# simzero/cudaParticlesFoam

Measured on AMD Instinct MI355X. Metric: Mparticle-steps/s, higher is better.
Workload: dtype f64

## Files before the change

### cudaparticlesfoam_amd/csrc/cpf_stream.hip

```cpp
#include "cpf_stream_ops.h"

#include <hip/hip_ext.h>

#include <type_traits>

namespace cpf {

#ifndef CPF_STREAM_SLOTS
#define CPF_STREAM_SLOTS 6
#endif
#ifndef CPF_STREAM_SLOTS_FIXED
#define CPF_STREAM_SLOTS_FIXED 9
#endif
#ifndef CPF_STREAM_WAVES
#define CPF_STREAM_WAVES 7
#endif
constexpr int kStreamSlots = CPF_STREAM_SLOTS;
constexpr int kStreamSlotsFixed = CPF_STREAM_SLOTS_FIXED;
constexpr int kSlotStride = 8;
static_assert(kStreamSlots >= 4 && kStreamSlots <= 32 && kStreamSlotsFixed >= 4 && kStreamSlotsFixed <= 32, "slots");
#ifndef CPF_STREAM_GATHER_LANES
#define CPF_STREAM_GATHER_LANES 32
#endif
constexpr int kStreamGatherLanes = CPF_STREAM_GATHER_LANES;
#ifndef CPF_STREAM_PAIRED
#define CPF_STREAM_PAIRED 0
#endif
#ifndef CPF_STREAM_INROUND
#define CPF_STREAM_INROUND 0
#endif
#ifndef CPF_STREAM_HIT_POOL
#define CPF_STREAM_HIT_POOL 40
#endif
constexpr int kVertexTets = 12;
#ifndef CPF_VERTEX_BLOCKS
#define CPF_VERTEX_BLOCKS 4
#endif
#ifndef CPF_VERTEX_PICK_UNROLL
#define CPF_VERTEX_PICK_UNROLL 12
#endif
constexpr int kVertexBlocks = CPF_VERTEX_BLOCKS;
constexpr int kStreamSparsePerCell = 8;
constexpr int kSitOut = INT32_MIN + 7;

struct StreamKernArgs {
    double *x, *y, *z; int32_t* cell; const int64_t* gid; double* vel; int64_t n; double dt, sigma; uint32_t step0; int nCyc;
    uint32_t seed; MeshView m; unsigned long long* counters; StreamArgs sa;
};
static_assert(offsetof(StreamKernArgs, x) == 0 && offsetof(StreamKernArgs, cell) == 24, "kernarg_cloud_ptrs reads bytes 0..31");
constexpr int kKernArgHitSpill = (int)(offsetof(StreamKernArgs, sa) + offsetof(StreamArgs, hitSpill));
constexpr int kKernArgZBad = (int)(offsetof(StreamKernArgs, sa) + offsetof(StreamArgs, zBad));
constexpr int kKernArgGid = (int)offsetof(StreamKernArgs, gid), kKernArgSigma = (int)offsetof(StreamKernArgs, sigma);
constexpr int kKernArgStep0 = (int)offsetof(StreamKernArgs, step0), kKernArgSeed = (int)offsetof(StreamKernArgs, seed);
#ifndef CPF_STREAM_BROWN_KERNARG
#define CPF_STREAM_BROWN_KERNARG 1
#endif

#ifndef CPF_STREAM_L1_ZERO_SKIP
#define CPF_STREAM_L1_ZERO_SKIP 1
#endif
#ifndef CPF_STREAM_LAZY_USED
#define CPF_STREAM_LAZY_USED 1
#endif
#ifndef CPF_STREAM_BOX_SPARSE
#define CPF_STREAM_BOX_SPARSE 1
#endif
#ifndef CPF_STREAM_FLAT_KICK
#define CPF_STREAM_FLAT_KICK 0
#endif
#ifndef CPF_STREAM_FLAT_ZERO_SKIP
#define CPF_STREAM_FLAT_ZERO_SKIP 0
#endif
#ifndef CPF_STREAM_FLAT_Z
#define CPF_STREAM_FLAT_Z 1
#endif
#ifndef CPF_STREAM_SLOTS_BOX
#define CPF_STREAM_SLOTS_BOX 9
#endif
#ifndef CPF_STREAM_SLOTS_BOX_B
#define CPF_STREAM_SLOTS_BOX_B 12
#endif
#ifndef CPF_STREAM_WAVES_BOX_B
#define CPF_STREAM_WAVES_BOX_B 6
#endif
#ifndef CPF_STREAM_WAVES_BOX
#define CPF_STREAM_WAVES_BOX 6
#endif
#ifndef CPF_STREAM_WAVES_B1
#define CPF_STREAM_WAVES_B1 5
#endif
#ifndef CPF_STREAM_WAVES_L2
#define CPF_STREAM_WAVES_L2 6
#endif
#ifndef CPF_STREAM_WAVES_B0
#define CPF_STREAM_WAVES_B0 7
#endif
#ifndef CPF_STREAM_HIT_POOL_B0
#define CPF_STREAM_HIT_POOL_B0 18
#endif
#ifndef CPF_STREAM_WAVES_FLAT
#define CPF_STREAM_WAVES_FLAT CPF_STREAM_WAVES
#endif
#ifndef CPF_STREAM_WAVES_FLAT_BODY
#define CPF_STREAM_WAVES_FLAT_BODY 0
#endif
template <bool BROWNIAN, bool STORE_VEL, bool STATS, int LOOKUP>
struct StreamOccupancy {
    static constexpr bool kMixed = LOOKUP == 2 || LOOKUP == 3 || LOOKUP == 5 || LOOKUP == 11;
    static constexpr int waves = (STORE_VEL || STATS) ? 1 : (LOOKUP == 4 ? (BROWNIAN ? 4 : 5) : (BROWNIAN ? (kMixed ? 5 : ((LOOKUP == 6 || LOOKUP == 11) ? CPF_STREAM_WAVES_BOX_B : (LOOKUP == 1 ? CPF_STREAM_WAVES_B1 : CPF_STREAM_WAVES_B0))) : (LOOKUP == 2 ? CPF_STREAM_WAVES_L2 : ((kMixed && LOOKUP != 11) ? 6 : ((LOOKUP == 6 || LOOKUP == 11) ? CPF_STREAM_WAVES_BOX : (LOOKUP == 8 ? CPF_STREAM_WAVES_FLAT : CPF_STREAM_WAVES))))));
};

template <bool BROWNIAN, bool REFLECT, bool STORE_VEL, bool STATS, int LOOKUP, bool VERTEX, bool ZSET = false>
__device__ __forceinline__ void stream_body(
    const int64_t* __restrict__ gid, double* __restrict__ vel, int64_t n, double dt, double sigma, uint32_t step0,
    int nCyc, uint32_t seed, const MeshView& m, unsigned long long* __restrict__ counters, const StreamArgs& sa, const VertexField& vf) {
#ifndef CPF_STREAM_SLOTS_BROWN
#define CPF_STREAM_SLOTS_BROWN 10
#endif
    constexpr int NS = (LOOKUP == 0 || LOOKUP == 5 || LOOKUP == 8) ? kStreamSlots : ((LOOKUP == 6 || LOOKUP == 11) ? (BROWNIAN ? CPF_STREAM_SLOTS_BOX_B : CPF_STREAM_SLOTS_BOX) : (BROWNIAN && LOOKUP == 1 ? CPF_STREAM_SLOTS_BROWN : kStreamSlotsFixed));
    constexpr bool BOX = LOOKUP == 6 || LOOKUP == 11;
    constexpr int kStride = BOX ? 4 : kSlotStride;
    constexpr unsigned kRecBytes = 32u * kStride;
    constexpr unsigned ALL = NS == 32 ? 0xFFFFFFFFu : ((1u << NS) - 1u);
    __shared__ double4 slots[NS][kStride];
    __shared__ unsigned sCnt[4];
#ifndef CPF_STREAM_HIT_REGS_L2
#define CPF_STREAM_HIT_REGS_L2 0
#endif
    constexpr bool HIT_IN_REGS = !BROWNIAN && (LOOKUP != 2 || CPF_STREAM_HIT_REGS_L2);
    constexpr bool kInRound = CPF_STREAM_INROUND == 2 || (CPF_STREAM_INROUND == 1 && BROWNIAN);
    static_assert(!(kInRound && (LOOKUP == 2 || LOOKUP == 3 || LOOKUP == 5 || LOOKUP == 11)), "in-round reflection knows neither face groups nor two-record cells");
    constexpr int kPool = HIT_IN_REGS ? 1 : ((LOOKUP == 2 || LOOKUP == 3 || LOOKUP == 5 || LOOKUP == 11) ? 16 : ((BROWNIAN && LOOKUP == 0) ? CPF_STREAM_HIT_POOL_B0 : CPF_STREAM_HIT_POOL));
    static_assert(!ZSET || ((LOOKUP == 8 || LOOKUP == 9) && !BROWNIAN && !VERTEX), "settled z: the flat walk without the kick or the vertex advect");
    __shared__ double sLane[ZSET ? 2 : 3][64];
    __shared__ double sPool[3][kPool];
    __shared__ unsigned sPoolUsed;
    __shared__ double sPre[ZSET ? 160 : (BROWNIAN ? 288 : 224)];
    __shared__ double sCone[VERTEX ? kVertexBlocks : 1][VERTEX ? kVertexTets * 10 : 1];
    double(*sE)[64] = sLane;
    const int lane = threadIdx.x;
    const unsigned ul = threadIdx.x;
    const unsigned preBase = uniform32(lds_addr(sPre));
    const unsigned slotBase = uniform32(lds_addr(slots));
    const int tpc = sa.tilesPerChunk;
    constexpr bool LOOKUP_FIXED = LOOKUP != 0 && LOOKUP != 5 && LOOKUP != 8;
    constexpr bool FLAT = LOOKUP == 8 || LOOKUP == 9;
    const bool zKeep = ZSET || (FLAT && CPF_STREAM_FLAT_Z != 0 && sa.zSettled != 0);
    auto park = [&](const D3& e) __attribute__((always_inline)) {
        sE[0][lane] = e.x; sE[1][lane] = e.y;
        if (!ZSET) sE[2][lane] = e.z;
    };
    auto parked = [&]() __attribute__((always_inline)) -> D3 {
        if (ZSET) return {sE[0][lane], sE[1][lane], 0.0};
        return {sE[0][lane], sE[1][lane], sE[2][lane]};
    };
    constexpr bool mixed = LOOKUP == 2 || LOOKUP == 3 || LOOKUP == 5 || LOOKUP == 11;
    constexpr bool bigCells = LOOKUP == 2;
    constexpr int kGatherAhead = LOOKUP == 4 ? 3 : 0;
    const bool zFold = !BOX && BROWNIAN && REFLECT && m.zThin != 0;
    const bool zLast = !FLAT && !BROWNIAN && m.zPairLast != 0;
    const bool flatKick = zFold && m.zSide0 != 0;
    const unsigned nTiles = (unsigned)((n + 63) >> 6);
    const unsigned nFull = (unsigned)(n >> 6), nTail = (unsigned)n & 63u;
    const unsigned big = sa.bigChunks;
    const unsigned nChunks = big + (nTiles - big * (unsigned)tpc);
    auto chunk_first = [&](unsigned c) -> unsigned {
        return c < big ? c * (unsigned)tpc : big * (unsigned)tpc + (c - big);
    };
    auto chunk_tiles = [&](unsigned c, unsigned firstTile) -> int {
        if (c >= nChunks) return 0;
        const unsigned k = nTiles - firstTile;
        const unsigned want = c < big ? (unsigned)tpc : 1u;
        return (int)(k < want ? k : want);
    };
    auto chunk_of = [&](unsigned j) -> unsigned {
        const unsigned long long c = (unsigned long long)(blockIdx.x & (kStreamGroups - 1)) + (unsigned long long)kStreamGroups * j;
        return c < (unsigned long long)nChunks ? (unsigned)c : nChunks;
    };
    StepStats st = {0, 0, 0, 0};
#ifdef CPF_STREAM_TIMELINE
    const uint64_t tl0 = __builtin_amdgcn_s_memrealtime();
    unsigned tlTiles = 0, tlRounds = 0;
    unsigned tlWaitRec = 0, tlWaitEnd = 0, tlMissRounds = 0;
    unsigned long long* const tlH = (!STORE_VEL && vel != nullptr && (sa.debug & 4)) ? reinterpret_cast<unsigned long long*>(vel) + 8 * 16384 : nullptr;
    unsigned tlVis = 0, tlRoundIdx = 0;
#endif

    for (unsigned k = blockIdx.x; k < (unsigned)kStreamGroups; k += gridDim.x)
        if (lane == 0) sa.grabNext[k * kStreamCounterStride] = 0u;
    const unsigned grp = blockIdx.x & (kStreamGroups - 1);
    unsigned* const myGrab = sa.grab + grp * kStreamCounterStride;

    auto prefetch = [&](unsigned t, const CloudPtrs& cp) __attribute__((always_inline)) -> int {
        double* const x = cp.x; double* const y = cp.y; double* const z = cp.z; int32_t* const cell = cp.cell;
        t = uniform32(t);
        const int64_t b = (int64_t)t * 64;
        unsigned ul = threadIdx.x;
        asm volatile("" : "+v"(ul));
        if (t < nFull) {
            const char* s1 = (ul < 32u ? reinterpret_cast<const char*>(x + b) : reinterpret_cast<const char*>(y + b)) + (ul & 31u) * 16u;
            glds16(s1, preBase);
            if (zKeep) {
                if (ul < 16u) glds16(reinterpret_cast<const char*>(cell + b) + ul * 16u, preBase + 1024u);
            } else if (ul < 48u) {
                const char* s2 = ul < 32u ? reinterpret_cast<const char*>(z + b) + ul * 16u
                                          : reinterpret_cast<const char*>(cell + b) + (ul - 32u) * 16u;
                glds16(s2, preBase + 1024u);
            }
            if (BROWNIAN) {
                const int64_t* const g = CPF_STREAM_BROWN_KERNARG ? static_cast<const int64_t*>(kernarg_pointer<kKernArgGid>()) : gid;
                if (g != nullptr) {
                    if (ul < 32u) glds16(reinterpret_cast<const char*>(g + b) + ul * 16u, preBase + 1792u);
                    return 3;
                }
            }
            return 2;
        }
        const unsigned lim = nTail - 1u;
        const unsigned l = ul < lim ? ul : lim;
        if (zKeep) {
            const double vx = (x + b)[l], vy = (y + b)[l];
            const int vc = (cell + b)[l];
            sPre[ul] = vx; sPre[64 + ul] = vy;
            reinterpret_cast<int*>(sPre + 128)[ul] = vc;
        } else {
        const double vx = (x + b)[l], vy = (y + b)[l], vz = (z + b)[l];
        const int vc = (cell + b)[l];
        sPre[ul] = vx; sPre[64 + ul] = vy; sPre[128 + ul] = vz;
        reinterpret_cast<int*>(sPre + 192)[ul] = vc;
        }
        if (BROWNIAN) {
            const int64_t* const g = CPF_STREAM_BROWN_KERNARG ? static_cast<const int64_t*>(kernarg_pointer<kKernArgGid>()) : gid;
            if (g != nullptr) reinterpret_cast<int64_t*>(sPre + 224)[ul] = (g + b)[l];
        }
        return 0;
    };

    unsigned got0 = 0;
    if (lane == 0) got0 = grab_sync(myGrab);
    const unsigned chunk0 = chunk_of(uniform32(got0));
    if (chunk_tiles(chunk0, chunk_first(chunk0)) > 0) {
        int tagv = -1;
        unsigned fifo = 0;

        unsigned tile = chunk_first(chunk0);
        int tilesLeft = chunk_tiles(chunk0, tile);
        (void)prefetch(tile, kernarg_cloud_ptrs());
        wait_vmcnt<0>();

        bool havePrev = false;
        unsigned rtile = 0;
        double rvx = 0, rvy = 0, rvz = 0;
        bool ralive = false;
        int rc = 0;
        unsigned rlim = 63;

        for (;;) {
            tile = uniform32(tile);
            const unsigned plim = tile < nFull ? 63u : nTail - 1u;
            double px = sPre[ul], py = sPre[64 + ul], pz = 0.0;
            int pc;
            if (zKeep) pc = reinterpret_cast<const int*>(sPre + 128)[ul];
            else { pz = sPre[128 + ul]; pc = reinterpret_cast<const int*>(sPre + 192)[ul]; }
            uint64_t pid = 0;
            if (BROWNIAN) {
                const bool haveIds = (CPF_STREAM_BROWN_KERNARG ? kernarg_pointer<kKernArgGid>() : (void*)gid) != nullptr;
                pid = haveIds ? (uint64_t) reinterpret_cast<const int64_t*>(sPre + 224)[ul] : (uint64_t)tile * 64 + ul;
            }
            if (ul > plim || pc < 0) pc = CPF_CELL_FROZEN;
            if (FLAT && !ZSET && !zKeep && ballot64(pc >= 0 && !(fabs(pz) <= 1.7976931348623157e308)) != 0ull) {
                unsigned* const bad = static_cast<unsigned*>(kernarg_pointer<kKernArgZBad>());
                if (bad != nullptr && lane == 0) *bad = 1u;
            }

            int cur = pc;
            int key2 = 0, carNext = 0, carBest = -1;
            double carDT = 2.0;
            D3 S_ = {px, py, pz}, v = {0, 0, 0};
            const uint64_t id = pid;

            unsigned ntile = 0;
            int ntilesLeft = 0;

            auto hook = [&](const D3& prev) __attribute__((always_inline)) -> int {
                int younger = 0;
                __builtin_amdgcn_sched_barrier(0);
                if (tilesLeft > 1) {
                    ntile = tile + 1;
                    ntilesLeft = tilesLeft - 1;
                } else {
                    unsigned got = 0;
                    if (lane == 0) got = grab_sync(myGrab);
                    const unsigned nxt = chunk_of(uniform32(got));
                    ntile = chunk_first(nxt);
                    ntilesLeft = chunk_tiles(nxt, ntile);
                }
                const CloudPtrs cp = kernarg_cloud_ptrs();
                double* const x = cp.x; double* const y = cp.y; double* const z = cp.z; int32_t* const cell = cp.cell;
                if (havePrev && !(sa.debug & 1)) {
                    const int64_t b = (int64_t)uniform32(rtile) * 64;
                    if (STORE_VEL && ralive) {
                        double* vv = vel + 3 * b;
                        async_store(vv, ul * 24u, rvx); async_store(vv + 1, ul * 24u, rvy); async_store(vv + 2, ul * 24u, rvz);
                    }
                    if (ul <= rlim) {
                        async_store(x + b, ul * 8u, prev.x); async_store(y + b, ul * 8u, prev.y);
                        if (!zKeep) async_store(z + b, ul * 8u, prev.z);
                        async_store(cell + b, ul * 4u, rc);
                    }
                    younger += zKeep ? 3 : 4;
                }
                if (ntilesLeft > 0 && !(sa.debug & 2)) younger += prefetch(ntile, cp);
                __builtin_amdgcn_sched_barrier(0);
                return younger;
            };

            bool busy = false;
            bool zUnclear = false;
            int token = INT32_MIN, h = 0, j = 0;
            int hitAt = -1;
            D3 hitReg = {0, 0, 0};
            auto park_hit = [&](const D3& Hp) __attribute__((always_inline)) {
                if (HIT_IN_REGS) { hitReg = Hp; return; }
                if (hitAt < 0) hitAt = (int)atomicAdd(&sPoolUsed, 1u);
                if (hitAt < kPool) { sPool[0][hitAt] = Hp.x; sPool[1][hitAt] = Hp.y; sPool[2][hitAt] = Hp.z; }
                else {
                    double* sp = static_cast<double*>(kernarg_pointer<kKernArgHitSpill>()) + (size_t)blockIdx.x * kStreamHitSpillDoubles;
                    async_store(sp, ul * 8u, Hp.x); async_store(sp + 64, ul * 8u, Hp.y); async_store(sp + 128, ul * 8u, Hp.z);
                }
            };

            auto cycle_begin = [&](int c) __attribute__((always_inline)) {
                if (cur < 0) cur = CPF_CELL_FROZEN;
                busy = cur >= 0;
                token = INT32_MIN; h = 0; j = 0;
                if (bigCells) key2 = 0;
                if (!HIT_IN_REGS && REFLECT) { hitAt = -1; if (lane == 0) sPoolUsed = 0u; }
                zUnclear = false;
                if (STATS && busy) ++st.steps;
                if (VERTEX) {
                    bool slow = busy;
#if defined(CPF_VERTEX_AB) && CPF_VERTEX_AB == 1
                    if (busy) { const double4 u = m.U[cur]; v = {u.x, u.y, u.z}; slow = false; }
#endif
                    if (vf.tetsPerCell == kVertexTets) {
                        unsigned long long todo = ballot64(slow);
                        while (todo != 0ull) {
                            int myBlock = -1;
                            __syncthreads();
#pragma unroll
                            for (int q = 0; q < kVertexBlocks; ++q) {
                                if (todo != 0ull) {
                                    const int ck = __builtin_amdgcn_readlane(cur, __ffsll((long long)todo) - 1);
                                    const bool mine = slow && cur == ck;
                                    if (mine) myBlock = q;
                                    if (lane < 5 * kVertexTets) {
                                        const int tk = lane / 5, piece = lane - 5 * tk;
                                        const double2 row = reinterpret_cast<const double2*>(vf.cone + kConeDoubles * ((int64_t)ck * kVertexTets + tk))[piece];
                                        reinterpret_cast<double2*>(&sCone[q][0] + 10 * tk)[piece] = row;
                                    }
                                    todo &= ~ballot64(mine);
                                }
                            }
                            __syncthreads();
                            if (myBlock >= 0) {
                                const double4 ap = vf.apex[cur];
                                const D3 A = {ap.x, ap.y, ap.z};
                                const D3 r = {S_.x - A.x, S_.y - A.y, S_.z - A.z};
                                int cand = 0;
                                double candMin = -1e300;
                                const double* blk = &sCone[myBlock][0];
#pragma unroll CPF_VERTEX_PICK_UNROLL
                                for (int k = 0; k < kVertexTets; ++k) {
                                    const double2* g = reinterpret_cast<const double2*>(blk + 10 * k);
                                    const double2 g01 = g[0], g23 = g[1], g45 = g[2], g67 = g[3], g89 = g[4];
                                    const double cb = fma(g23.x, r.z, fma(g01.y, r.y, g01.x * r.x)), cc = fma(g45.y, r.z, fma(g45.x, r.y, g23.y * r.x));
                                    const double cd = fma(g89.x, r.z, fma(g67.y, r.y, g67.x * r.x));
                                    const double mm = fmin(cb, fmin(cc, cd));
                                    if (mm > candMin) { candMin = mm; cand = k; }
                                }
#if defined(CPF_VERTEX_AB) && CPF_VERTEX_AB == 2
                                { const double4 u = m.U[cur]; v = {u.x + 1e-300 * cand, u.y, u.z}; slow = false; }
#else
                                D3 vv;
                                if (vertex_velocity_in_tet(vf, S_, A, (int64_t)cur * kVertexTets + cand, vv)) { v = vv; slow = false; }
#endif
                            }
                        }
                    }
                    if (slow) (void)vertex_velocity(vf, S_, cur, v);
                }
            };

            auto round = [&](bool hookDue, bool cycleStart, int c) __attribute__((always_inline)) {
#ifdef CPF_STREAM_TIMELINE
                ++tlRounds;
                bool tlSat = false;
#endif
                const unsigned long long busyMask = ballot64(busy);
                const D3 Epre = parked();
                const int lk = (bigCells && key2 != 0) ? key2 : cur;
                int myslot = -1;
                unsigned used = 0;
                unsigned long long missLanes = busyMask;
                if (LOOKUP_FIXED) {
                    const int cell0 = __builtin_amdgcn_readlane(lk, __ffsll((long long)busyMask) - 1);
                    const unsigned long long in0 = __builtin_amdgcn_uicmp((unsigned)lk, (unsigned)cell0, 32 ) & busyMask;
                    if (in0 == busyMask) {
                        const unsigned long long hitTag = __builtin_amdgcn_uicmp((unsigned)tagv, (unsigned)cell0, 32 ) & ALL;
                        if (hitTag != 0ull) {
                            myslot = __ffsll((long long)hitTag) - 1;
                            used = (unsigned)hitTag;
                            missLanes = 0ull;
                        }
                    } else {
#if CPF_STREAM_LAZY_USED
                        unsigned long long eqs[NS];
#pragma unroll
                        for (int k = 0; k < NS; ++k) {
                            const int tk = __builtin_amdgcn_readlane(tagv, k);
                            eqs[k] = __builtin_amdgcn_uicmp((unsigned)lk, (unsigned)tk, 32 );
                            asm("v_cndmask_b32_e64 %0, %1, %2, %3" : "=v"(myslot) : "v"(myslot), "n"(k), "s"(eqs[k]));
                        }
                        missLanes = ballot64(myslot < 0) & busyMask;
                        if (missLanes != 0ull) {
#pragma unroll
                            for (int k = 0; k < NS; ++k) used |= ((eqs[k] & busyMask) != 0ull ? 1u : 0u) << k;
                        }
#else
#pragma unroll
                        for (int k = 0; k < NS; ++k) {
                            const int tk = __builtin_amdgcn_readlane(tagv, k);
                            const unsigned long long eqK = __builtin_amdgcn_uicmp((unsigned)lk, (unsigned)tk, 32 );
                            const unsigned long long inK = eqK & busyMask;
                            asm("v_cndmask_b32_e64 %0, %1, %2, %3" : "=v"(myslot) : "v"(myslot), "n"(k), "s"(eqK));
                            used |= (inK != 0ull ? 1u : 0u) << k;
                            missLanes &= ~inK;
                        }
#endif
                    }
                } else {
                    unsigned long long todo = busyMask;
                    missLanes = 0ull;
                    while (todo != 0ull) {
                        const int leader = __ffsll((long long)todo) - 1;
                        const int ck = __builtin_amdgcn_readlane(lk, leader);
                        const bool mine = lk == ck;
                        const unsigned long long same = ballot64(mine) & busyMask;
                        const unsigned long long hitTag = __builtin_amdgcn_uicmp((unsigned)tagv, (unsigned)ck, 32 );
                        if (hitTag != 0ull) {
                            const int sl = __ffsll((long long)hitTag) - 1;
                            used |= 1u << sl;
                            if (mine) myslot = sl;
                        } else {
                            missLanes |= same;
                        }
                        todo &= ~same;
                    }
                }
                int nJobs = 0;
                if (missLanes != 0ull) {
#define CPF_JOB(J)                                                                                          \
                    if (missLanes != 0ull && used != ALL) {                                                 \
                        const int leader = __ffsll((long long)missLanes) - 1;                               \
                        const int ck = __builtin_amdgcn_readlane(lk, leader);                               \
                        const unsigned cand = ~used & ALL;                                                  \
                        const unsigned hi = cand & (ALL << fifo) & ALL;                                     \
                        const int victim = __ffs((int)(hi ? hi : cand)) - 1;                                \
                        fifo = (unsigned)(victim + 1) == (unsigned)NS ? 0u : (unsigned)(victim + 1);          \
                        used |= 1u << victim;                                                               \
                        if (lane == victim) tagv = ck;                                                      \
                        const bool mine = lk == ck;                                                         \
                        if (mine) myslot = victim;                                                          \
                        missLanes &= ~ballot64(mine);                                                       \
                        if (ul < kRecBytes / 16u)                                                            \
                            glds16(reinterpret_cast<const char*>(BOX ? m.boxRec : m.cellRec) + (int64_t)ck * kRecBytes + ul * 16u,  \
                                   uniform32(slotBase + (unsigned)victim * kRecBytes));                     \
                        nJobs = J + 1;                                                                      \
                    }
                    CPF_JOB(0) CPF_JOB(1) CPF_JOB(2) CPF_JOB(3)
                    if (LOOKUP_FIXED) { CPF_JOB(4) CPF_JOB(5) CPF_JOB(6) CPF_JOB(7) }
#undef CPF_JOB
                }
                int younger = 0;
                if (hookDue) younger = hook(Epre);
                if (BROWNIAN && cycleStart && busy) {
                    uint32_t kStep0 = step0, kSeed = seed;
                    if (CPF_STREAM_BROWN_KERNARG) kernarg_u32_pair<kKernArgStep0, kKernArgSeed>(kStep0, kSeed);
                    const D3 xi = normal3(id, kStep0 + (uint32_t)c, kSeed);
                    sE[0][lane] = xi.x; sE[1][lane] = xi.y; sE[2][lane] = xi.z;
                }
#ifdef CPF_STREAM_TIMELINE
                const uint64_t tlw0 = __builtin_amdgcn_s_memrealtime();
#endif
                if (nJobs != 0) {
                    if (ZSET) {
                        if (younger == 5) wait_vmcnt<5>();
                        else if (younger == 3) wait_vmcnt<3>();
                        else if (younger == 2) wait_vmcnt<2>();
                        else wait_vmcnt<0>();
                    } else
                    if (younger >= 7) wait_vmcnt<7>();
                    else if (younger == 6) wait_vmcnt<6>();
                    else if (younger == 5) wait_vmcnt<5>();
                    else if (younger >= 4) wait_vmcnt<4>();
                    else if (younger == 3) wait_vmcnt<3>();
                    else if (younger >= 2) wait_vmcnt<2>();
                    else wait_vmcnt<0>();
#ifdef CPF_STREAM_TIMELINE
                    tlWaitRec += (unsigned)(__builtin_amdgcn_s_memrealtime() - tlw0); ++tlMissRounds;
#endif
                }
                const bool gatherRound = __popcll(missLanes) >= kStreamGatherLanes;
                auto advect = [&](const double4* rec) __attribute__((always_inline)) -> D3 {
                    D3 Pn;
                    if (VERTEX) {
                        Pn = {S_.x + dt * v.x, S_.y + dt * v.y, S_.z + dt * v.z};
                    } else {
                        double4 u;
                        if (BOX) { const double2 uxy = reinterpret_cast<const double2*>(rec)[5]; u = {uxy.x, uxy.y, reinterpret_cast<const double*>(rec)[12], 0.0}; }
                        else u = rec[6];
                        v = {u.x, u.y, u.z};
                        if (ZSET) Pn = {fma(dt, v.x, S_.x), fma(dt, v.y, S_.y), 0.0};
                        else Pn = axpy(dt, v, S_);
                    }
                    D3 disp = {Pn.x - S_.x, Pn.y - S_.y, ZSET ? 0.0 : Pn.z - S_.z};
                    if (BROWNIAN) {
                        const D3 xi = {sE[0][lane], sE[1][lane], sE[2][lane]};
                        disp = axpy(CPF_STREAM_BROWN_KERNARG ? kernarg_f64<kKernArgSigma>() : sigma, xi, disp);
                    }
                    D3 E = {S_.x + disp.x, S_.y + disp.y, ZSET ? 0.0 : S_.z + disp.z};
                    if (BROWNIAN && REFLECT && zFold) {
                        bool clear;
                        const int nb = fold_z(E.z, rec[BOX ? 0 : 4], rec[BOX ? 0 : 5], clear);
                        zUnclear |= ballot64(!clear) != 0ull;
                        if (STATS) st.refl += nb;
                        if (STORE_VEL && (nb & 1)) v.z = -v.z;
                    }
                    park(E);
                    return E;
                };
                if (busy) {
                    int next, outSlot = 0;
                    double4 wallPlane;
                    const bool needAdvect = token == INT32_MIN && !(bigCells && key2 != 0);
                    D3 E = S_;
                    if (!needAdvect) E = Epre;
                    bool hdrCell = false;
                    if (bigCells && myslot >= 0) hdrCell = *reinterpret_cast<const int*>(&slots[0][0] + myslot * kSlotStride + 7) == kBigCellMark;
                    if (myslot >= 0 && !(bigCells && hdrCell)) {
                        const double4* rec = &slots[0][0] + myslot * kStride;
                        if (needAdvect) E = advect(rec);
                        bool twoRec = false;
                        int recB = 0;
                        const bool second0 = key2 != 0;
                        if (bigCells) {
                            const int2 cont = reinterpret_cast<const int2*>(rec + 7)[3];
                            twoRec = !second0 && cont.x == kTwoRecMark;
                            recB = cont.y;
                        }
                        bool again;
                        do {
                            again = false;
                            if (bigCells) {
                                const D3 P0 = S_;
                                const D3 Pd = {E.x - P0.x, E.y - P0.y, E.z - P0.z};
                                double dTm = second0 ? carDT : 2.0;
                                int nx = second0 ? carNext : cur, bs = second0 ? carBest : -1;
                                trace_lds6_record<!BROWNIAN, mixed>(P0, Pd, rec, token, second0 ? 6 : 0, dTm, nx, bs);
                                if (twoRec) {
                                    carDT = dTm; carNext = nx; carBest = bs;
                                    key2 = recB;
                                    next = kSitOut;
                                } else {
                                    key2 = 0;
                                    if (bs >= 0) { S_ = axpy(dTm, Pd, P0); outSlot = bs; }
                                    next = nx;
                                    if (STATS) ++st.hops;
                                }
                            } else {
                            if (BOX) next = trace_box<!BROWNIAN, mixed>(S_, E, cur, rec, token, outSlot);
                            else if (FLAT) next = trace_lds4_flat<(CPF_STREAM_FLAT_ZERO_SKIP != 0)>(S_, E, cur, rec, token, outSlot);
                            else if (CPF_STREAM_FLAT_KICK && BROWNIAN && !mixed && flatKick && !zUnclear)
                            next = trace_lds4_flat_z<false>(S_, E, cur, rec, token, outSlot);
                            else
                            next = (CPF_STREAM_PAIRED && LOOKUP_FIXED && !BROWNIAN && !mixed) ? trace_lds6_paired(S_, E, cur, rec, token, outSlot, zLast)
                                                                : trace_lds6<(!BROWNIAN && (CPF_STREAM_L1_ZERO_SKIP || LOOKUP != 1)), mixed>(S_, E, cur, rec, token, outSlot, zLast, zFold && !zUnclear);
                            if (STATS) ++st.hops;
                            }
                            if (REFLECT && next < 0 && !(mixed && is_group(next))) {
                                if (bigCells && lk != cur) {
                                    if (outSlot >= 6) wallPlane = rec[outSlot - 6];
                                    else {
                                        wallPlane = m.planes[m.cellOff[cur] + outSlot];
                                        asm volatile("" : "+v"(wallPlane.x), "+v"(wallPlane.y), "+v"(wallPlane.z), "+v"(wallPlane.w));
                                    }
                                } else if (BOX) wallPlane = box_wall_plane(rec, outSlot);
                                else wallPlane = rec[outSlot];
                                asm volatile("" ::: "memory");
                                E = parked();
                                if (kInRound) {
                                    park_hit(S_);
                                    if (STATS) ++st.refl;
                                    const D3 nn = {wallPlane.x, wallPlane.y, wallPlane.z};
                                    const double sd = dot3(wallPlane, E) - wallPlane.w;
                                    E = axpy(-2.0 * sd, nn, E);
                                    sE[0][lane] = E.x; sE[1][lane] = E.y; sE[2][lane] = E.z;
                                    v = axpy(-2.0 * dot3(wallPlane, v), nn, v);
                                    token = next;
                                    h = 0;
                                    if (++j == kMaxReflect) { busy = false; next = cur; }
                                    else again = true;
                                }
                            }
                        } while (again);
                    } else {
                        next = kSitOut;
                        if (gatherRound || (bigCells && hdrCell)) {
                            const double4* rec = BOX ? m.boxRec + 4 * (int64_t)cur : m.cellRec + 8 * (int64_t)cur;
                            if (needAdvect) E = advect(rec);
                            int gS0 = 0;
                            bool gBig = false;
                            if (LOOKUP_FIXED && bigCells) {
                                const int4 hdr = *reinterpret_cast<const int4*>(rec + 7);
                                const int2 cont = reinterpret_cast<const int2*>(rec + 7)[3];
                                gBig = hdr.x == kBigCellMark || cont.x == kTwoRecMark;
                                if (gBig) {
                                    gS0 = m.cellOff[cur];
                                    next = trace_csr(S_, E, cur, m.planes, m.nbr, gS0, m.cellOff[cur + 1] - gS0, token, outSlot);
                                    rec = m.planes + gS0;
                                    key2 = 0;
                                }
                            }
                            if (BOX) next = trace_box<false, mixed>(S_, E, cur, rec, token, outSlot);
                            else if (!gBig)
                            next = trace_fixed<6, false, mixed, kGatherAhead>(S_, E, cur, rec, reinterpret_cast<const int32_t*>(rec + 7), token, outSlot, 0);
                            if (STATS) ++st.hops;
                            if (REFLECT && next < 0) {
                                wallPlane = BOX ? box_wall_plane(rec, outSlot) : rec[outSlot];
                                asm volatile("" : "+v"(wallPlane.x), "+v"(wallPlane.y), "+v"(wallPlane.z), "+v"(wallPlane.w));
                            }
                        }
                    }
                    if (mixed && next != kSitOut && is_group(next)) next = resolve_group(next, S_, m.cellOff, m.planes, m.groupOff, m.groupNbr);
#ifdef CPF_STREAM_TIMELINE
                    if (next == kSitOut) tlSat = true; else ++tlVis;
#endif
                    const bool ends = next == cur;
                    const bool wall = next < 0 && next != kSitOut;
                    const bool cross = next >= 0 && !ends;
                    if (wall) {
                        if (!REFLECT) j = kMaxReflect;
                        else {
                            park_hit(S_);
                            if (STATS) ++st.refl;
                            const D3 nn = {wallPlane.x, wallPlane.y, wallPlane.z};
                            const double sd = (ZSET ? fma(wallPlane.y, E.y, wallPlane.x * E.x) : dot3(wallPlane, E)) - wallPlane.w;
                            if (ZSET) E = {fma(-2.0 * sd, nn.x, E.x), fma(-2.0 * sd, nn.y, E.y), 0.0};
                            else E = axpy(-2.0 * sd, nn, E);
                            park(E);
                            v = axpy(-2.0 * dot3(wallPlane, v), nn, v);
                            h = 0;
                            ++j;
                        }
                    }
                    token = cross ? cur : (wall ? next : token);
                    cur = cross ? next : cur;
                    h += cross ? 1 : 0;
                    busy = !(ends || (cross && h == kMaxHops) || (wall && j >= kMaxReflect));
                }
#ifdef CPF_STREAM_TIMELINE
                {
                    const unsigned nb = (unsigned)__popcll(busyMask), ns = (unsigned)__popcll(ballot64(tlSat));
                    const unsigned r = tlRoundIdx < 15u ? tlRoundIdx : 15u;
                    if (tlH != nullptr && lane == 0) {
                        atomicAdd(&tlH[r * 65u + nb], 1ull); atomicAdd(&tlH[16 * 65 + r], (unsigned long long)ns);
                        atomicAdd(&tlH[16 * 65 + 16 + 256 + r], (unsigned long long)nJobs);
                    }
                    ++tlRoundIdx;
                }
#endif
            };

            auto cycle_end = [&]() __attribute__((always_inline)) {
                if (cur >= 0) {
                    const D3 E = parked();
                    if (REFLECT && j != 0) {
                        D3 hit;
                        if (HIT_IN_REGS) hit = hitReg;
                        else if (hitAt < kPool) hit = {sPool[0][hitAt], sPool[1][hitAt], sPool[2][hitAt]};
                        else load3_sync(static_cast<const double*>(kernarg_pointer<kKernArgHitSpill>()) + (size_t)blockIdx.x * kStreamHitSpillDoubles,
                                        ul * 8u, hit.x, hit.y, hit.z);
                        S_ = {hit.x + (E.x - hit.x), hit.y + (E.y - hit.y), ZSET ? 0.0 : hit.z + (E.z - hit.z)};
                    } else S_ = E;
                    if (j >= kMaxReflect) { cur = CPF_CELL_LOST; if (STATS) ++st.lost; }
                }
            };

            if (nCyc > 0) {
                for (int c = 0; c < nCyc; ++c) {
                    cycle_begin(c);
#ifdef CPF_STREAM_TIMELINE
                    tlVis = 0; tlRoundIdx = 0;
#endif
                    bool hookDue = c == 0, cycleStart = true;
#ifdef CPF_STREAM_CAP_TEST
                    int capRounds = 0, capLimit = CPF_STREAM_CAP_TEST;
                    asm volatile("" : "+s"(capLimit));
                    do { round(hookDue, cycleStart, c); hookDue = false; cycleStart = false; ++capRounds; } while (ballot64(busy) != 0ull && capRounds < capLimit);
                    const bool capDropped = busy;
                    const D3 capKeep = S_;
                    const int capCur = cur;
#else
                    do { round(hookDue, cycleStart, c); hookDue = false; cycleStart = false; } while (ballot64(busy) != 0ull);
#endif
#ifdef CPF_STREAM_TIMELINE
                    {
                        unsigned mx = tlVis;
                        for (int off = 32; off > 0; off >>= 1) { const unsigned o = (unsigned)__shfl_xor((int)mx, off, 64); mx = o > mx ? o : mx; }
                        const unsigned r = tlRoundIdx < 15u ? tlRoundIdx : 15u, iv = mx < 15u ? mx : 15u;
                        if (tlH != nullptr && lane == 0) atomicAdd(&tlH[16 * 65 + 16 + r * 16u + iv], 1ull);
                    }
#endif
                    cycle_end();
#ifdef CPF_STREAM_CAP_TEST
                    if (capDropped) { S_ = capKeep; cur = capCur; }
#endif
                }
            } else {
                const D3 prev = parked();
                (void)hook(prev);
            }

#ifdef CPF_STREAM_TIMELINE
            const uint64_t tle0 = __builtin_amdgcn_s_memrealtime();
#endif
            wait_vmcnt<0>();
#ifdef CPF_STREAM_TIMELINE
            tlWaitEnd += (unsigned)(__builtin_amdgcn_s_memrealtime() - tle0);
            ++tlTiles;
#endif
            rtile = tile; havePrev = true;
            park(S_);
            if (STORE_VEL) { rvx = v.x; rvy = v.y; rvz = v.z; ralive = pc >= 0; }
            rc = cur;
            rlim = plim;
            if (ntilesLeft <= 0) break;
            tile = ntile; tilesLeft = ntilesLeft;
        }
        {
            const int64_t b = (int64_t)rtile * 64;
            const CloudPtrs cp = kernarg_cloud_ptrs();
            double* const x = cp.x; double* const y = cp.y; double* const z = cp.z; int32_t* const cell = cp.cell;
            const D3 res = parked();
            if (ul <= rlim) {
                (x + b)[ul] = res.x; (y + b)[ul] = res.y;
                if (!zKeep) (z + b)[ul] = res.z;
                (cell + b)[ul] = rc;
            }
            if (STORE_VEL && ralive) {
                double* vv = vel + 3 * b;
                vv[3 * ul] = rvx; vv[3 * ul + 1] = rvy; vv[3 * ul + 2] = rvz;
            }
        }
    }
#ifdef CPF_STREAM_TIMELINE
    if (!STORE_VEL && vel != nullptr && lane == 0) {
        uint64_t* o = reinterpret_cast<uint64_t*>(vel) + 8 * (uint64_t)blockIdx.x;
        o[0] = tl0; o[1] = __builtin_amdgcn_s_memrealtime(); o[2] = tlTiles; o[3] = tlRounds;
        o[4] = tlWaitRec; o[5] = tlWaitEnd; o[6] = tlMissRounds; o[7] = 0;
    }
#endif
    if (STATS) flush_stats(st, counters, sCnt);
}

template <bool BROWNIAN, bool REFLECT, bool STORE_VEL, bool STATS, int LOOKUP>
__global__ __launch_bounds__(64, (StreamOccupancy<BROWNIAN, STORE_VEL, STATS, LOOKUP>::waves)) void step_kernel_stream(
    double* __restrict__ , double* __restrict__ , double* __restrict__ , int32_t* __restrict__ ,
    const int64_t* __restrict__ gid, double* __restrict__ vel, int64_t n, double dt, double sigma, uint32_t step0,
    int nCyc, uint32_t seed, MeshView m, unsigned long long* __restrict__ counters, StreamArgs sa) {
    stream_body<BROWNIAN, REFLECT, STORE_VEL, STATS, LOOKUP, false>(gid, vel, n, dt, sigma, step0, nCyc, seed, m, counters, sa, VertexField{});
}

#ifndef CPF_STREAM_WAVES_VERTEX
#define CPF_STREAM_WAVES_VERTEX 4
#endif
template <bool BROWNIAN, bool REFLECT, bool STORE_VEL, bool STATS, int LOOKUP>
__global__ __launch_bounds__(64, ((STORE_VEL || STATS) ? 1 : CPF_STREAM_WAVES_VERTEX)) void step_kernel_stream_vertex(
    double* __restrict__ , double* __restrict__ , double* __restrict__ , int32_t* __restrict__ ,
    const int64_t* __restrict__ gid, double* __restrict__ vel, int64_t n, double dt, double sigma, uint32_t step0,
    int nCyc, uint32_t seed, MeshView m, unsigned long long* __restrict__ counters, StreamArgs sa, VertexField vf) {
    stream_body<BROWNIAN, REFLECT, STORE_VEL, STATS, LOOKUP, true>(gid, vel, n, dt, sigma, step0, nCyc, seed, m, counters, sa, vf);
}

template <bool REFLECT, bool STORE_VEL, bool STATS, int LOOKUP>
__global__ __launch_bounds__(64, (StreamOccupancy<false, STORE_VEL, STATS, LOOKUP>::waves)) void step_kernel_stream_flat(
    double* __restrict__ , double* __restrict__ , double* __restrict__ , int32_t* __restrict__ ,
    const int64_t* __restrict__ gid, double* __restrict__ vel, int64_t n, double dt, double sigma, uint32_t step0,
    int nCyc, uint32_t seed, MeshView m, unsigned long long* __restrict__ counters, StreamArgs sa) {
    stream_body<false, REFLECT, STORE_VEL, STATS, LOOKUP, false, true>(gid, vel, n, dt, sigma, step0, nCyc, seed, m, counters, sa, VertexField{});
}

template <bool B, bool R_, bool SV, bool ST, int LF, bool VX = false, bool ZS = false>
static hipError_t launch_stream_inst(hipStream_t st, double* x, double* y, double* z, int32_t* cell, const int64_t* gid,
                                     double* vel, int64_t n, double dt, double sigma, uint32_t step0, int nCyc,
                                     uint32_t seed, const MeshView& m, unsigned long long* counters, StreamState& ss,
                                     const VertexField* vf, bool settled, hipEvent_t evStart, hipEvent_t evStop) {
    static int wavesPerCU = 0;
    if (wavesPerCU == 0) {
        int nb = 0;
        hipError_t e;
        if constexpr (VX) e = hipOccupancyMaxActiveBlocksPerMultiprocessor(&nb, step_kernel_stream_vertex<B, R_, SV, ST, LF>, 64, 0);
        else if constexpr (ZS) e = hipOccupancyMaxActiveBlocksPerMultiprocessor(&nb, step_kernel_stream_flat<R_, SV, ST, LF>, 64, 0);
        else e = hipOccupancyMaxActiveBlocksPerMultiprocessor(&nb, step_kernel_stream<B, R_, SV, ST, LF>, 64, 0);
        if (e != hipSuccess) return e;
        wavesPerCU = nb < 1 ? 1 : (nb > 32 ? 32 : nb);
        if (ZS && CPF_STREAM_WAVES_FLAT_BODY > 0 && wavesPerCU > 4 * CPF_STREAM_WAVES_FLAT_BODY) wavesPerCU = 4 * CPF_STREAM_WAVES_FLAT_BODY;
    }
    const int64_t nTiles = (n + 63) >> 6;
    if (nTiles >= ((int64_t)1 << 31)) return hipErrorInvalidValue;
    const int64_t slotsOnChip = (int64_t)((ss.wavesPerCU > 0 && !VX) ? ss.wavesPerCU : wavesPerCU) * ss.numCU;
    int tpc = ss.tilesPerChunk > 0 ? ss.tilesPerChunk : ((LF == 0 || LF == 5 || LF == 8) ? 4 : 3);
    const double tailFraction = ss.tailFraction >= 0.0 ? ss.tailFraction : ((LF == 0 || LF == 5 || LF == 8) ? 0.1 : 0.2);
    while (tpc > 1 && nTiles / tpc < 4 * slotsOnChip) tpc = tpc > 2 ? tpc - 1 : 1;
    int64_t bigChunks = (int64_t)((double)(nTiles / tpc) * (1.0 - tailFraction));
    if (tpc == 1 || bigChunks < 0) bigChunks = 0;
    const int64_t nChunks = bigChunks + (nTiles - bigChunks * tpc);
    int64_t R = slotsOnChip / kStreamGroups;
    const int64_t need = (nChunks + kStreamGroups - 1) / kStreamGroups;
    if (R > need) R = need;
    if (R < 1) R = 1;
    unsigned* cur = ss.d_grab + (size_t)(ss.parity & 1) * kStreamGroups * kStreamCounterStride;
    unsigned* nxt = ss.d_grab + (size_t)((ss.parity & 1) ^ 1) * kStreamGroups * kStreamCounterStride;
    if (R * kStreamGroups > ss.hitSpillWaves) R = ss.hitSpillWaves / kStreamGroups;
    if (R < 1 || ss.d_hitSpill == nullptr) return hipErrorInvalidValue;
    const bool zSettled = (LF == 8 || LF == 9) && !VX && settled && ss.flatZ != 0;
    if (ZS != zSettled && (LF == 8 || LF == 9) && !VX) return hipErrorInvalidValue;
    StreamArgs sa = {cur, nxt, (int)R, tpc, (unsigned)bigChunks, ss.debug, ss.d_hitSpill, zSettled ? 1 : 0, ss.zBad};
    if constexpr (VX) {
        if (vf == nullptr) return hipErrorInvalidValue;
        if (evStart != nullptr && evStop != nullptr)
            hipExtLaunchKernelGGL((step_kernel_stream_vertex<B, R_, SV, ST, LF>), dim3((unsigned)(R * kStreamGroups)), dim3(64), 0, st, evStart,
                                  evStop, 0, x, y, z, cell, gid, vel, n, dt, sigma, step0, nCyc, seed, m, counters, sa, *vf);
        else
        hipLaunchKernelGGL((step_kernel_stream_vertex<B, R_, SV, ST, LF>), dim3((unsigned)(R * kStreamGroups)), dim3(64), 0, st, x, y, z, cell,
                           gid, vel, n, dt, sigma, step0, nCyc, seed, m, counters, sa, *vf);
        return stream_launch_done(st, ss);
    } else if constexpr (ZS) {
        if (evStart != nullptr && evStop != nullptr)
            hipExtLaunchKernelGGL((step_kernel_stream_flat<R_, SV, ST, LF>), dim3((unsigned)(R * kStreamGroups)), dim3(64), 0, st, evStart,
                                  evStop, 0, x, y, z, cell, gid, vel, n, dt, sigma, step0, nCyc, seed, m, counters, sa);
        else
        hipLaunchKernelGGL((step_kernel_stream_flat<R_, SV, ST, LF>), dim3((unsigned)(R * kStreamGroups)), dim3(64), 0, st, x, y, z, cell,
                           gid, vel, n, dt, sigma, step0, nCyc, seed, m, counters, sa);
        return stream_launch_done(st, ss);
    } else {
    if (evStart != nullptr && evStop != nullptr)
        hipExtLaunchKernelGGL((step_kernel_stream<B, R_, SV, ST, LF>), dim3((unsigned)(R * kStreamGroups)), dim3(64), 0, st, evStart,
                              evStop, 0, x, y, z, cell, gid, vel, n, dt, sigma, step0, nCyc, seed, m, counters, sa);
    else
    hipLaunchKernelGGL((step_kernel_stream<B, R_, SV, ST, LF>), dim3((unsigned)(R * kStreamGroups)), dim3(64), 0, st, x, y, z, cell,
                       gid, vel, n, dt, sigma, step0, nCyc, seed, m, counters, sa);
    return stream_launch_done(st, ss);
    }
}

static int stream_lookup_mode(int64_t n, const MeshView& m, const StreamState& ss, bool brown, bool vertex) {
    int64_t cells = m.nCells;
    if (ss.densityLookup && ss.occupiedHost != nullptr) {
        const int64_t occ = (int64_t)ss.occupiedHost[0], live = (int64_t)ss.occupiedHost[1];
        if (occ > 0 && occ <= cells && live > 0 && live <= 2 * n && n <= 2 * live) cells = occ;
    }
    if (vertex) return n < 128 * cells ? 1 : 0;
    if (m.mixed == 1 && m.boxRec != nullptr && m.zThin == 0 && ss.lookup < 0) return 11;
    if (m.mixed) return m.mixed == 2 ? 2 : ((ss.lookup >= 0 ? ss.lookup == 0 : n >= 128 * cells) ? 5 : 3);
    const bool box = m.boxRec != nullptr && m.zThin == 0;
    if (ss.lookup >= 0) return (ss.lookup == 6 && !box) ? 1 : ss.lookup;
    if (box && CPF_STREAM_BOX_SPARSE) return 6;
    if (n < kStreamSparsePerCell * cells) return 4;
    const bool flat = !brown && ss.flat && ss.flatField && m.zSide0 != 0;
    if (n < 128 * cells) return flat ? 9 : 1;
    return flat ? 8 : 0;
}

StepPlan plan_step(const MeshView& m, const StreamState& ss, int variant, const VertexField* vf, int64_t n, int nCyc, double D,
                   unsigned flags, bool stats) {
    StepPlan p;
    p.brown = D > 0.0;
    p.reflect = (flags & CPF_STEP_NO_REFLECT) == 0;
    p.storeVel = (flags & CPF_STEP_STORE_VEL) != 0;
    p.stats = stats;
    const int coopMaxCells = (ss.coopMaxCells <= 0 || ss.coopMaxCells > kCoopMaxCells) ? kCoopMaxCells : ss.coopMaxCells;
    if (!m.allHex) {
        const bool wantsStream = variant == kVariantAuto || variant == kVariantStream || variant == kVariantCoop;
        variant = (m.mixed && m.cellRec && wantsStream) ? kVariantStream : kVariantGeneric;
    } else {
        if (variant == kVariantAuto)
            variant = !(nCyc >= kFusedCoopCycles && m.nCells <= coopMaxCells) ? kVariantStream : kVariantCoop;
        if (variant == kVariantCoop && m.nCells > coopMaxCells) variant = kVariantStream;
#ifndef CPF_EXPERIMENTS
        if (variant == kVariantFixed || variant == kVariantFixedScalar) variant = kVariantCoop;
        if (variant == kVariantAhead) variant = kVariantStream;
#endif
    }
    if (vf != nullptr) {
        p.cone = vf->cone != nullptr;
        const bool streams = p.cone && vf->tetsPerCell == 12 && m.mixed == 0 && m.cellRec != nullptr && variant == kVariantStream;
        p.kernel = streams ? StepPlan::kStreamVertex : StepPlan::kVertex;
        if (streams) p.lookup = stream_lookup_mode(n, m, ss, p.brown, true);
        return p;
    }
    if (variant == kVariantAhead && (p.brown || p.storeVel || nCyc != 1)) variant = kVariantStream;
    p.kernel = (StepPlan::Kernel)variant;
    if (variant == kVariantStream) p.lookup = stream_lookup_mode(n, m, ss, p.brown, false);
    return p;
}

template <int... L, class F>
static hipError_t with_lookup(int lookup, F&& f) {
    hipError_t e = hipErrorInvalidValue;
    (void)((lookup == L && ((e = f(std::integral_constant<int, L>{})), true)) || ...);
    return e;
}
hipError_t launch_step_stream(const StepPlan& p, hipStream_t st, double* x, double* y, double* z, int32_t* cell, const int64_t* gid,
                              double* vel, int64_t n, double dt, double sigma, uint32_t step0, int nCyc, uint32_t seed,
                              const MeshView& m, unsigned long long* counters, const VertexField* vf, StreamState& ss, bool zSettled,
                              hipEvent_t evStart, hipEvent_t evStop) {
    return with_bools([&](auto B, auto R, auto SV, auto ST) {
        if (p.kernel == StepPlan::kStreamVertex)
            return with_lookup<0, 1>(p.lookup, [&](auto LF) {
                return launch_stream_inst<B, R, SV, ST, LF, true>(st, x, y, z, cell, gid, vel, n, dt, sigma, step0, nCyc, seed, m,
                                                                  counters, ss, vf, zSettled, evStart, evStop);
            });
        if (p.flat_body(ss, zSettled))
            return with_lookup<8, 9>(p.lookup, [&](auto LF) {
                if constexpr (B) return hipErrorInvalidValue;
                else return launch_stream_inst<false, R, SV, ST, LF, false, true>(st, x, y, z, cell, gid, vel, n, dt, sigma, step0, nCyc, seed, m,
                                                                                  counters, ss, vf, zSettled, evStart, evStop);
            });
        return with_lookup<0, 1, 2, 3, 4, 5, 6, 8, 9, 11>(p.lookup, [&](auto LF) {
            if constexpr (B && (LF == 8 || LF == 9)) return hipErrorInvalidValue;
            else return launch_stream_inst<B, R, SV, ST, LF>(st, x, y, z, cell, gid, vel, n, dt, sigma, step0, nCyc, seed, m, counters,
                                                             ss, vf, zSettled, evStart, evStop);
        });
    }, p.brown, p.reflect, p.storeVel, p.stats);
}

}
```

Before: 105,800.

## Streamline settled-z flat walk round: wave-mask busy, hints, flat gather, single hook path

For the settled-z flat lookup specialization, the change keeps the busy state as a wave-wide 64-bit mask and restores per-lane busy with an inverse ballot. It also adds branch-likelihood hints, a dedicated flat gather trace for off-slot cells, and non-short-circuit busy arithmetic. The zero-cycle hook path is merged into the main loop so there is a single round instantiation, and unrolling of the round loop is disabled. The aim is less control flow, fewer SGPR/VGPR conversions and smaller code in the hot round loop. The risks are changed register pressure, and the hint path drops the big-cell header check, which only holds because the flat lookup has no big cells.

```diff
diff --git a/cudaparticlesfoam_amd/csrc/cpf_stream.hip b/cudaparticlesfoam_amd/csrc/cpf_stream.hip
--- a/cudaparticlesfoam_amd/csrc/cpf_stream.hip
+++ b/cudaparticlesfoam_amd/csrc/cpf_stream.hip
@@ -103,6 +103,21 @@
 #endif
 #ifndef CPF_STREAM_WAVES_FLAT_BODY
 #define CPF_STREAM_WAVES_FLAT_BODY 0
+#endif
+#ifndef CPF_FLAT_ROUND_GATHER
+#define CPF_FLAT_ROUND_GATHER 1
+#endif
+#ifndef CPF_FLAT_ROUND_HINTS
+#define CPF_FLAT_ROUND_HINTS 1
+#endif
+#ifndef CPF_FLAT_ROUND_ONE_HOOK
+#define CPF_FLAT_ROUND_ONE_HOOK 1
+#endif
+#ifndef CPF_FLAT_ROUND_MASK
+#define CPF_FLAT_ROUND_MASK 1
+#endif
+#ifndef CPF_FLAT_ROUND_OUTCOME
+#define CPF_FLAT_ROUND_OUTCOME 1
 #endif
 template <bool BROWNIAN, bool STORE_VEL, bool STATS, int LOOKUP>
 struct StreamOccupancy {
@@ -145,6 +160,9 @@
     const int tpc = sa.tilesPerChunk;
     constexpr bool LOOKUP_FIXED = LOOKUP != 0 && LOOKUP != 5 && LOOKUP != 8;
     constexpr bool FLAT = LOOKUP == 8 || LOOKUP == 9;
+    constexpr bool kMaskBusy = ZSET && CPF_FLAT_ROUND_MASK != 0, kPlainOutcome = ZSET && CPF_FLAT_ROUND_OUTCOME != 0;
+    constexpr bool kFlatGather = ZSET && CPF_FLAT_ROUND_GATHER != 0, kHints = ZSET && CPF_FLAT_ROUND_HINTS != 0;
+    constexpr bool kOneHook = ZSET && CPF_FLAT_ROUND_ONE_HOOK != 0;
     const bool zKeep = ZSET || (FLAT && CPF_STREAM_FLAT_Z != 0 && sa.zSettled != 0);
     auto park = [&](const D3& e) __attribute__((always_inline)) {
         sE[0][lane] = e.x; sE[1][lane] = e.y;
@@ -316,6 +334,7 @@
             };
 
             bool busy = false;
+            unsigned long long busyM = 0ull;
             bool zUnclear = false;
             int token = INT32_MIN, h = 0, j = 0;
             int hitAt = -1;
@@ -333,6 +352,7 @@
             auto cycle_begin = [&](int c) __attribute__((always_inline)) {
                 if (cur < 0) cur = CPF_CELL_FROZEN;
                 busy = cur >= 0;
+                if (kMaskBusy) busyM = ballot64(cur >= 0);
                 token = INT32_MIN; h = 0; j = 0;
                 if (bigCells) key2 = 0;
                 if (!HIT_IN_REGS && REFLECT) { hitAt = -1; if (lane == 0) sPoolUsed = 0u; }
@@ -397,7 +417,8 @@
                 ++tlRounds;
                 bool tlSat = false;
 #endif
-                const unsigned long long busyMask = ballot64(busy);
+                const unsigned long long busyMask = kMaskBusy ? busyM : ballot64(busy);
+                if (kMaskBusy) busy = __builtin_amdgcn_inverse_ballot_w64(busyM);
                 const D3 Epre = parked();
                 const int lk = (bigCells && key2 != 0) ? key2 : cur;
                 int myslot = -1;
@@ -548,7 +569,7 @@
                     if (!needAdvect) E = Epre;
                     bool hdrCell = false;
                     if (bigCells && myslot >= 0) hdrCell = *reinterpret_cast<const int*>(&slots[0][0] + myslot * kSlotStride + 7) == kBigCellMark;
-                    if (myslot >= 0 && !(bigCells && hdrCell)) {
+                    if ((kHints && __builtin_expect(myslot >= 0, 1)) || (!kHints && myslot >= 0 && !(bigCells && hdrCell))) {
                         const double4* rec = &slots[0][0] + myslot * kStride;
                         if (needAdvect) E = advect(rec);
                         bool twoRec = false;
@@ -616,7 +637,7 @@
                         } while (again);
                     } else {
                         next = kSitOut;
-                        if (gatherRound || (bigCells && hdrCell)) {
+                        if ((kHints && __builtin_expect(gatherRound, 0)) || (!kHints && (gatherRound || (bigCells && hdrCell)))) {
                             const double4* rec = BOX ? m.boxRec + 4 * (int64_t)cur : m.cellRec + 8 * (int64_t)cur;
                             if (needAdvect) E = advect(rec);
                             int gS0 = 0;
@@ -633,6 +654,7 @@
                                 }
                             }
                             if (BOX) next = trace_box<false, mixed>(S_, E, cur, rec, token, outSlot);
+                            else if (kFlatGather) next = trace_lds4_flat<false>(S_, E, cur, rec, token, outSlot);
                             else if (!gBig)
                             next = trace_fixed<6, false, mixed, kGatherAhead>(S_, E, cur, rec, reinterpret_cast<const int32_t*>(rec + 7), token, outSlot, 0);
                             if (STATS) ++st.hops;
@@ -667,8 +689,11 @@
                     token = cross ? cur : (wall ? next : token);
                     cur = cross ? next : cur;
                     h += cross ? 1 : 0;
+                    if (kPlainOutcome) busy = !(ends | (cross & (h == kMaxHops)) | (wall & (j >= kMaxReflect)));
+                    else
                     busy = !(ends || (cross && h == kMaxHops) || (wall && j >= kMaxReflect));
                 }
+                if (kMaskBusy) busyM = ballot64(busy);
 #ifdef CPF_STREAM_TIMELINE
                 {
                     const unsigned nb = (unsigned)__popcll(busyMask), ns = (unsigned)__popcll(ballot64(tlSat));
@@ -697,9 +722,12 @@
                 }
             };
 
-            if (nCyc > 0) {
-                for (int c = 0; c < nCyc; ++c) {
-                    cycle_begin(c);
+            const int nRun = (kOneHook && nCyc <= 0) ? 1 : nCyc;
+            if (kOneHook || nCyc > 0) {
+                for (int c = 0; c < nRun; ++c) {
+                    int live = nCyc;
+                    if (kOneHook) asm volatile("" : "+s"(live));
+                    if (live > 0) cycle_begin(c);
 #ifdef CPF_STREAM_TIMELINE
                     tlVis = 0; tlRoundIdx = 0;
 #endif
@@ -712,6 +740,10 @@
                     const D3 capKeep = S_;
                     const int capCur = cur;
 #else
+                    if constexpr (ZSET) {
+                        _Pragma("clang loop unroll(disable)")
+                        do { round(hookDue, cycleStart, c); hookDue = false; cycleStart = false; } while (kMaskBusy ? busyM != 0ull : ballot64(busy) != 0ull);
+                    } else
                     do { round(hookDue, cycleStart, c); hookDue = false; cycleStart = false; } while (ballot64(busy) != 0ull);
 #endif
 #ifdef CPF_STREAM_TIMELINE
@@ -722,7 +754,7 @@
                         if (tlH != nullptr && lane == 0) atomicAdd(&tlH[16 * 65 + 16 + r * 16u + iv], 1ull);
                     }
 #endif
-                    cycle_end();
+                    if (live > 0) cycle_end();
 #ifdef CPF_STREAM_CAP_TEST
                     if (capDropped) { S_ = capKeep; cur = capCur; }
 #endif
```

Result: faster. 109,500, median of 6 (+3.5%).
